# wanmeihuali/taichi_3d_gaussian_splatting

Hardware: NVIDIA B200
Metric: rendered Mpix/sec fwd+bwd @1080p, 1e6 Gaussians (higher is better)
Workload: dtype f32

## Files before the change

taichi_3d_gaussian_splatting_b200/csrc/api.cu:

```cuda
#include <cstdarg>
#include <cstdio>
#include <cstring>

#include "common.cuh"

namespace gsb {

static thread_local char g_error[512] = "";

void set_error(const char *fmt, ...) {
    va_list ap;
    va_start(ap, fmt);
    vsnprintf(g_error, sizeof(g_error), fmt, ap);
    va_end(ap);
}

static inline int64_t align_up(int64_t v, int64_t a) { return (v + a - 1) / a * a; }

static int bit_width(uint64_t v) {
    int b = 0;
    while (v) {
        ++b;
        v >>= 1;
    }
// ... 73 lines not shown
                      int32_t H, int32_t W, float far_plane, float depth_scale, uint32_t flags,
                      Workspace *ws) {
    int rc = compute_layout(N, n_obj, key_capacity, H, W, far_plane, depth_scale, flags, &ws->layout);
    if (rc != GSB_OK) return rc;
    const GsbWorkspaceLayout &L = ws->layout;
    if (!base || bytes < L.total_bytes) {
        set_error("workspace too small: have %lld bytes, need %lld", (long long)bytes, (long long)L.total_bytes);
        return GSB_EWORKSPACE;
    }
    if (reinterpret_cast<uintptr_t>(base) % 256 != 0) {
        set_error("workspace must be 256-byte aligned");
        return GSB_EINVAL;
    }
    char *b = static_cast<char *>(base);
    ws->counters = reinterpret_cast<long long *>(b + L.counters);
    ws->tickets = reinterpret_cast<unsigned int *>(b + L.tickets);
    ws->scan_state = reinterpret_cast<unsigned long long *>(b + L.scan_state);
    ws->sort_hist = reinterpret_cast<unsigned int *>(b + L.sort_hist);
    ws->sort_state = reinterpret_cast<unsigned int *>(b + L.sort_state);
    ws->tile_start = reinterpret_cast<int *>(b + L.tile_start);
    ws->tile_end = reinterpret_cast<int *>(b + L.tile_end);
    ws->poses = reinterpret_cast<PoseBlock *>(b + L.poses);
    ws->point_id = reinterpret_cast<int *>(b + L.point_id);
    ws->point_offset = reinterpret_cast<int *>(b + L.point_offset);
    ws->num_tiles = reinterpret_cast<int *>(b + L.num_tiles);
    ws->records = reinterpret_cast<float4 *>(b + L.records);
    ws->point_in_camera = reinterpret_cast<float *>(b + L.point_in_camera);
    ws->keys_a = b + L.keys_a;
    ws->keys_b = b + L.keys_b;
    ws->vals_a = reinterpret_cast<int *>(b + L.vals_a);
    ws->vals_b = reinterpret_cast<int *>(b + L.vals_b);
    ws->keys_c = b + L.keys_c;
    ws->vals_c = reinterpret_cast<int *>(b + L.vals_c);
    return GSB_OK;
}

static int check_forward_args(const GsbForwardArgs *a) {
    if (!a) {
        set_error("forward: args is null");
        return GSB_EINVAL;
    }
    if (a->num_points > 0 && (!a->pointcloud || !a->pointcloud_features || !a->point_invalid_mask ||
                              !a->point_object_id)) {
        set_error("forward: null scene pointer");
        return GSB_EINVAL;
    }
    if (a->num_points > 0 && (a->num_objects <= 0 || !a->q_pointcloud_camera || !a->t_pointcloud_camera)) {
        set_error("forward: need at least one object pose");
        return GSB_EINVAL;
    }
    if (!a->camera_intrinsics || !a->rasterized_image) {
        set_error("forward: null camera_intrinsics / rasterized_image");
        return GSB_EINVAL;
    }
    if (!a->rgb_only && (!a->rasterized_depth || !a->pixel_accumulated_alpha ||
                         !a->pixel_offset_of_last_effective_point || !a->pixel_valid_point_count)) {
        set_error("forward: aux outputs are required unless rgb_only");
        return GSB_EINVAL;
    }
    if (a->near_plane < 0.0f) {
        set_error("forward: near_plane must be >= 0 (depth keys are unsigned)");
        return GSB_EUNSUPPORTED;
    }
    if (reinterpret_cast<uintptr_t>(a->pointcloud_features) % 16 != 0) {
        set_error("forward: pointcloud_features must be 16-byte aligned");
        return GSB_EINVAL;
// ... 435 lines not shown
```

taichi_3d_gaussian_splatting_b200/csrc/blend_bwd.cu:

```cuda
#include "blend_bwd.cuh"

namespace gsb {

__device__ __forceinline__ void warp_transpose_reduce11(float (&v)[11], int lane) {
    {
        const bool hi = lane & 16;
#pragma unroll
        for (int i = 0; i < 5; ++i) {
            const float send = hi ? v[i] : v[i + 6];
            const float keep = hi ? v[i + 6] : v[i];
            v[i] = keep + __shfl_xor_sync(0xffffffffu, send, 16);
        }
        v[5] += __shfl_xor_sync(0xffffffffu, v[5], 16);
    }
    {
        const bool hi = lane & 8;
#pragma unroll
        for (int i = 0; i < 3; ++i) {
            const float send = hi ? v[i] : v[i + 3];
            const float keep = hi ? v[i + 3] : v[i];
            v[i] = keep + __shfl_xor_sync(0xffffffffu, send, 8);
        }
    }
    {
// ... 185 lines not shown
            }
        }
    }
    if (STATS) {
        p.mag_image[2 * pix] = mag0;
        p.mag_image[2 * pix + 1] = mag1;
    }
}

#ifndef GSB_HOST_EMU
static BlendBwdParams make_blend_bwd_params(const GsbBackwardArgs &a, const Workspace &ws);

int launch_blend_backward_work(const GsbBackwardArgs &a, const Workspace &ws, unsigned long long *counters_dev,
                               cudaStream_t stream) {
    BlendBwdParams p = make_blend_bwd_params(a, ws);
    p.work_counters = counters_dev;
    const int tiles = p.tiles_x * (a.camera_height / GSB_TILE_HEIGHT);
    if (tiles <= 0) return GSB_OK;
    return launch_blend_backward_count(p, tiles, stream);
}

static BlendBwdParams make_blend_bwd_params(const GsbBackwardArgs &a, const Workspace &ws) {
    BlendBwdParams p;
    p.H = a.camera_height;
    p.W = a.camera_width;
    p.tiles_x = a.camera_width / GSB_TILE_WIDTH;
    p.tile_start = ws.tile_start;
    p.tile_end = ws.tile_end;
    p.sorted_vals = ws.vals_b;
    p.records = ws.records;
    p.grad_image = a.grad_rasterized_image;
    p.acc_alpha = a.pixel_accumulated_alpha;
    p.last_effective = a.pixel_offset_of_last_effective_point;
    p.accum = a.accum;
    p.mag_image = a.magnitude_grad_viewspace_on_image;
    p.work_counters = nullptr;
    return p;
}

int launch_blend_backward(const GsbBackwardArgs &a, const Workspace &ws, cudaStream_t stream) {
    BlendBwdParams p;
    p.H = a.camera_height;
    p.W = a.camera_width;
    p.tiles_x = a.camera_width / GSB_TILE_WIDTH;
    p.tile_start = ws.tile_start;
    p.tile_end = ws.tile_end;
    p.sorted_vals = ws.vals_b;
    p.records = ws.records;
    p.grad_image = a.grad_rasterized_image;
    p.acc_alpha = a.pixel_accumulated_alpha;
    p.last_effective = a.pixel_offset_of_last_effective_point;
    p.accum = a.accum;
    p.mag_image = a.magnitude_grad_viewspace_on_image;
    p.work_counters = nullptr;
    const int tiles = p.tiles_x * (a.camera_height / GSB_TILE_HEIGHT);
    if (tiles <= 0) return GSB_OK;
    if (a.flags & GSB_FLAG_BACKWARD_TRANSPOSED)
        return launch_blend_backward_transposed(p, tiles, (a.flags & GSB_FLAG_EXACT_EXP) != 0,
                                                (a.flags & GSB_FLAG_NO_HOOK_STATS) == 0, stream);
    const bool exact = (a.flags & GSB_FLAG_EXACT_EXP) != 0;
    if (a.flags & GSB_FLAG_NO_HOOK_STATS) {
        if (exact) blend_backward_kernel<true, false><<<tiles, GSB_TILE_PIXELS, 0, stream>>>(p);
        else blend_backward_kernel<false, false><<<tiles, GSB_TILE_PIXELS, 0, stream>>>(p);
    } else if (exact) {
        blend_backward_kernel<true><<<tiles, GSB_TILE_PIXELS, 0, stream>>>(p);
    } else {
        blend_backward_kernel<false><<<tiles, GSB_TILE_PIXELS, 0, stream>>>(p);
    }
    GSB_CUDA_CHECK(cudaGetLastError());
    return GSB_OK;
}
#endif

__device__ __forceinline__ void sh_basis(float dx, float dy, float dz, float (&sh)[16]) {
    const float dinv = 1.0f / sqrtf(dx * dx + dy * dy + dz * dz);
    dx *= dinv; dy *= dinv; dz *= dinv;
    sh[0] = 0.28209479177387814f;
    sh[1] = -0.48860251190291987f * dy;
    sh[2] = 0.48860251190291987f * dz;
    sh[3] = -0.48860251190291987f * dx;
    sh[4] = 1.0925484305920792f * dx * dy;
    sh[5] = -1.0925484305920792f * dy * dz;
    sh[6] = 0.94617469575755997f * dz * dz - 0.31539156525251999f;
    sh[7] = -1.0925484305920792f * dx * dz;
// ... 368 lines not shown
```

taichi_3d_gaussian_splatting_b200/csrc/blend_bwd.cuh:

```cuda
#pragma once
#include "common.cuh"

namespace gsb {

struct BlendBwdParams {
    int H, W, tiles_x;
    const int *tile_start;
    const int *tile_end;
    const int *sorted_vals;
    const float4 *records;
    const float *grad_image;
    const float *acc_alpha;
    const int *last_effective;
    float *accum;
    float *mag_image;
    unsigned long long *work_counters;
};

#ifdef GSB_HOST_EMU
__device__ __forceinline__ float ex2_approx_b(float x) { return exp2f(x); }
__device__ __forceinline__ float rcp_approx(float x) { return 1.0f / x; }
__device__ __forceinline__ float sqrt_approx(float x) { return sqrtf(x); }
#else
__device__ __forceinline__ float ex2_approx_b(float x) {
    float y;
    asm("ex2.approx.ftz.f32 %0, %1;" : "=f"(y) : "f"(x));
    return y;
}
__device__ __forceinline__ float rcp_approx(float x) {
    float y;
    asm("rcp.approx.ftz.f32 %0, %1;" : "=f"(y) : "f"(x));
    return y;
}
__device__ __forceinline__ float sqrt_approx(float x) {
    float y;
    asm("sqrt.approx.ftz.f32 %0, %1;" : "=f"(y) : "f"(x));
    return y;
}
#endif

int launch_blend_backward_transposed(const BlendBwdParams &p, int tiles, bool exact_exp, bool stats,
                                     cudaStream_t stream);
int launch_blend_backward_count(const BlendBwdParams &p, int tiles, cudaStream_t stream);

}
```

taichi_3d_gaussian_splatting_b200/csrc/blend_bwd_transposed.cu:

```cuda
#include "blend_bwd.cuh"

namespace gsb {

constexpr int TB_CHUNK = 16;
constexpr int TB_ROW = TB_CHUNK + 1;
constexpr int TB_TR_ROW = 13;

struct TbShared {
    float4 rec[2 * 3 * GSB_TILE_PIXELS];
    float4 g[8][32];
    float xg[8][32 * TB_ROW];
    float xa[8][32 * TB_ROW];
    int off[2][GSB_TILE_PIXELS];
    float4 chunk[8][3][TB_CHUNK];
    int chunk_off[8][TB_CHUNK];
    unsigned int bits[2][8][8];
    unsigned char list[8][GSB_TILE_PIXELS];
    int max_last;
};
static_assert(32 * TB_ROW >= TB_CHUNK * TB_TR_ROW, "finished rows must fit into the exchange buffer");

#ifdef GSB_HOST_EMU
static inline unsigned char *tb_dynamic_smem() { return simt_emu::dynamic_smem(); }
#else
extern __shared__ __align__(16) unsigned char gsb_tb_dynamic_smem[];
__device__ __forceinline__ unsigned char *tb_dynamic_smem() { return gsb_tb_dynamic_smem; }
#endif

#ifndef GSB_TB_P1_UNROLL
#define GSB_TB_P1_UNROLL 4
#endif
constexpr int TB_P1_UNROLL = GSB_TB_P1_UNROLL;
#ifndef GSB_TB_MIN_BLOCKS
#define GSB_TB_MIN_BLOCKS 3
#endif
__device__ __forceinline__ float keep_if_contributing(float P, int idx, int last) {
#ifdef GSB_HOST_EMU
    return ((idx < last) && (P >= 1.0f / 255.0f)) ? P : 0.0f;
#else
    float r;
    asm("{\n"
        ".reg .pred p, q;\n"
        "setp.lt.s32 q, %2, %3;\n"
        "setp.ge.and.f32 p, %1, 0f3B808081, q;\n"
        "selp.f32 %0, %1, 0f00000000, p;\n"
        "}\n"
        : "=f"(r)
        : "f"(P), "r"(idx), "r"(last));
    return r;
#endif
}

template <bool EXACT_EXP, bool STATS, bool COUNT = false>
__global__ void __launch_bounds__(GSB_TILE_PIXELS, GSB_TB_MIN_BLOCKS)
blend_backward_transposed_kernel(const BlendBwdParams p) {
    TbShared &S = *reinterpret_cast<TbShared *>(tb_dynamic_smem());
    constexpr int NV = STATS ? 11 : 9;

    const int tile = blockIdx.x;
    const int tu = tile % p.tiles_x, tv = tile / p.tiles_x;
    const int tid = threadIdx.x, lane = tid & 31, warp = tid >> 5;
    const int pu = tu * GSB_TILE_WIDTH + (warp & 1) * 8 + (lane & 7);
    const int pv = tv * GSB_TILE_HEIGHT + (warp >> 1) * 4 + (lane >> 3);
    const float px = (float)pu + 0.5f, py = (float)pv + 0.5f;
    const float tile_x0 = (float)(tu * GSB_TILE_WIDTH), tile_y0 = (float)(tv * GSB_TILE_HEIGHT);
    const size_t pix = (size_t)pv * p.W + pu;
    const int start = p.tile_start[tile];

    const int last = p.last_effective[pix];
    float T = 1.0f - p.acc_alpha[pix];
    float w0 = 0.0f, w1 = 0.0f, w2 = 0.0f;
    const float g0 = p.grad_image[3 * pix], g1 = p.grad_image[3 * pix + 1], g2 = p.grad_image[3 * pix + 2];
    float mag0 = 0.0f, mag1 = 0.0f;
    unsigned int n_visits = 0, n_pairs = 0;
    S.g[warp][lane] = make_float4(g0, g1, g2, 0.0f);

    const int ci = lane & (TB_CHUNK - 1), half = lane >> 4;
    const float pxb = tile_x0 + (float)((warp & 1) * 8) + 0.5f;
    const float pyb = tile_y0 + (float)((warp >> 1) * 4 + 2 * half) + 0.5f;
    float *const xg = S.xg[warp], *const xa = S.xa[warp];
    const int fl_row = lane >= GSB_ACCUM_FLOATS ? 1 : 0;
    const int fl_word = lane - GSB_ACCUM_FLOATS * fl_row;
    const bool fl_ok = lane < 2 * GSB_ACCUM_FLOATS && fl_word < NV;
    const int *const fl_off = S.chunk_off[warp] + fl_row;
    const float *const fl_val = xg + fl_row * TB_TR_ROW + (fl_ok ? fl_word : 0);
    unsigned char *const list = S.list[warp];

    int warp_last = last;
#pragma unroll
    for (int d = 16; d > 0; d >>= 1) warp_last = max(warp_last, __shfl_xor_sync(0xffffffffu, warp_last, d));
    if (tid == 0) S.max_last = start;
    __syncthreads();
    if (lane == 0) atomicMax(&S.max_last, warp_last);
    __syncthreads();
    const int end = min(p.tile_end[tile], S.max_last);

    float4 *const ck0 = S.chunk[warp][0], *const ck1 = S.chunk[warp][1], *const ck2 = S.chunk[warp][2];
    int *const ck_off = S.chunk_off[warp];
    int have = 0;

    int buf = 0;
    for (int block_end = end;; block_end -= GSB_TILE_PIXELS, buf ^= 1) {
        const bool real = block_end > start;
        int count = 0;
        float4 *const s_r0 = S.rec + buf * 3 * GSB_TILE_PIXELS;
        float4 *const s_r1 = s_r0 + GSB_TILE_PIXELS, *const s_r2 = s_r0 + 2 * GSB_TILE_PIXELS;
        if (real) {
            const int block_start = max(block_end - GSB_TILE_PIXELS, start);
            {
                const int idx = block_end - 1 - tid;
                unsigned int mask = 0;
                if (idx >= block_start) {
                    const int o = __ldg(&p.sorted_vals[idx]);
                    const float4 *rec = p.records + 3 * (size_t)o;
                    const float4 r0 = __ldg(rec), r1 = __ldg(rec + 1);
                    if (EXACT_EXP) {
                        s_r0[tid] = r0;
                        s_r1[tid] = r1;
                    } else {
                        float4 f0, f1;
                        fast_planes(r0, r1, f0, f1);
                        s_r0[tid] = f0;
                        s_r1[tid] = f1;
                    }
                    s_r2[tid] = __ldg(rec + 2);
                    S.off[buf][tid] = o;
                    mask = splat_patch_mask(r0.x, r0.y, r0.z, r0.w, r1.x, r1.y * r1.z, tile_x0, tile_y0);
                }
#pragma unroll
                for (int w = 0; w < 8; ++w) {
                    const unsigned int bits = __ballot_sync(0xffffffffu, (mask >> w) & 1u);
                    if (lane == 0) S.bits[buf][w][warp] = bits;
                }
            }
            __syncthreads();
            if (tid == 0) GSB_EMU_COUNT(EC_BATCHES, 1);
            if (block_start < warp_last) {
                const int skip = block_end - warp_last;
#pragma unroll
                for (int k = 0; k < 8; ++k) {
                    unsigned int bits = S.bits[buf][warp][k];
                    const int lo = skip - 32 * k;
                    if (lo >= 32) bits = 0u;
                    else if (lo > 0) bits &= ~((1u << lo) - 1u);
                    if ((bits >> lane) & 1u)
                        list[count + __popc(bits & ((1u << lane) - 1u))] = (unsigned char)(k * 32 + lane);
                    count += __popc(bits);
                }
                __syncwarp();
            }
        }

        int pos = 0;
#pragma unroll 1
        do {
            if (pos < count) {
                const int take = min(TB_CHUNK - have, count - pos);
                if (lane < take) {
                    const int j = list[pos + lane], slot = have + lane;
                    ck0[slot] = s_r0[j];
                    ck1[slot] = s_r1[j];
                    float4 r2 = s_r2[j];
                    r2.w = __int_as_float(block_end - 1 - j);
                    ck2[slot] = r2;
                    ck_off[slot] = S.off[buf][j];
                }
                have += take;
                pos += take;
                __syncwarp();
            }
            if (have == TB_CHUNK || (!real && have > 0)) {
                const int n = have;
                have = 0;
                if (COUNT) n_visits += (lane == 0) ? (unsigned int)n : 0u;
                if (lane == 0) {
                    GSB_EMU_COUNT(EC_TB_SPLATS, n);
                    GSB_EMU_COUNT(EC_TB_CHUNKS, 1);
                }
#pragma unroll TB_P1_UNROLL
                for (int i = 0; i < n; ++i) {
                    const float4 r0 = ck0[i];
                    const float4 r1 = ck1[i];
                    const float4 r2 = ck2[i];
                    const int idx = __float_as_int(r2.w);
                    const float d0 = px - r0.x, d1 = py - r0.y;
                    float G, aT;
                    if (EXACT_EXP) {
                        const float q0 = r0.z * d0 + r0.w * d1;
                        const float q1 = r0.w * d0 + r1.x * d1;
                        const float gp = expf(-0.5f * (d0 * q0 + d1 * q1)) * r1.y;
                        const float prod_alpha = gp * r1.z;
                        const bool contributes = (idx < last) && (prod_alpha >= 1.0f / 255.0f);
                        const float alpha = fminf(prod_alpha, 0.99f);
                        const float inv = 1.0f / (1.0f - alpha);
                        const float Tn = T * inv;
                        aT = contributes ? alpha * Tn : 0.0f;
                        const float a_grad = contributes ? (r2.x * Tn - w0 * inv) * g0 + (r2.y * Tn - w1 * inv) * g1 +
                                                               (r2.z * Tn - w2 * inv) * g2
                                                         : 0.0f;
                        T = contributes ? Tn : T;
                        w0 = fmaf(r2.x, aT, w0);
                        w1 = fmaf(r2.y, aT, w1);
                        w2 = fmaf(r2.z, aT, w2);
                        G = a_grad * r1.z * gp;
                        if (STATS) {
                            mag0 += fabsf(G * q0);
                            mag1 += fabsf(G * q1);
                        }
                    } else {
                        float P = fast_alpha(d0, d1, r0.z, r0.w, r1.x, r1.y);
                        P = keep_if_contributing(P, idx, last);
                        const float alpha = fminf(P, 0.99f);
                        const float inv = rcp_approx(1.0f - alpha);
                        T *= inv;
                        aT = alpha * T;
                        const float cg = fmaf(r2.z, g2, fmaf(r2.y, g1, r2.x * g0));
                        const float a_grad = fmaf(cg, T, -(w0 * inv));
                        w0 = fmaf(cg, aT, w0);
                        G = a_grad * P;
                        if (STATS) {
                            const float q0 = (-2.0f / GSB_L2E) * fmaf(r0.z, d0, 0.5f * r0.w * d1);
                            const float q1 = (-2.0f / GSB_L2E) * fmaf(0.5f * r0.w, d0, r1.x * d1);
                            mag0 += fabsf(G * q0);
                            mag1 += fabsf(G * q1);
                        }
                    }
                    if (COUNT) n_pairs += aT > 0.0f ? 1u : 0u;
                    xg[lane * TB_ROW + i] = G;
                    xa[lane * TB_ROW + i] = aT;
                }
                __syncwarp();

                const bool active = ci < n;
                float4 s0 = ck0[active ? ci : 0];
                float4 s1 = ck1[active ? ci : 0];
                if (!EXACT_EXP) {
                    s0.z *= -2.0f / GSB_L2E;
                    s0.w *= -1.0f / GSB_L2E;
                    s1.x *= -2.0f / GSB_L2E;
                }
                const float dx0 = pxb - s0.x;
                float acc[11];
#pragma unroll
                for (int k = 0; k < 11; ++k) acc[k] = 0.0f;
                unsigned int nz = 0u;
#pragma unroll
                for (int row = 0; row < 2; ++row) {
                    const float d1 = (pyb + (float)row) - s0.y;
                    float q0 = s0.z * dx0 + s0.w * d1;
                    float q1 = s0.w * dx0 + s1.x * d1;
#pragma unroll
                    for (int k = 0; k < 8; ++k) {
                        const int pp = 8 * row + k + 16 * half;
                        const float G = xg[pp * TB_ROW + ci], aT = xa[pp * TB_ROW + ci];
                        const float4 gp = S.g[warp][pp];
                        const float vs0 = G * q0, vs1 = G * q1;
                        acc[0] += vs0;
                        acc[1] += vs1;
                        acc[2] = fmaf(vs0, q0, acc[2]);
                        acc[3] = fmaf(vs0, q1, acc[3]);
                        acc[4] = fmaf(vs1, q1, acc[4]);
                        acc[5] = fmaf(aT, gp.x, acc[5]);
                        acc[6] = fmaf(aT, gp.y, acc[6]);
                        acc[7] = fmaf(aT, gp.z, acc[7]);
                        acc[8] += G;
                        if (STATS) {
                            const float m2 = vs0 * vs0 + vs1 * vs1;
                            acc[9] += EXACT_EXP ? sqrtf(m2) : sqrt_approx(m2);
                            acc[10] += aT > 0.0f ? 1.0f : 0.0f;
                        }
                        nz |= __float_as_uint(aT);
                        q0 += s0.z;
                        q1 += s0.w;
                    }
                }
#pragma unroll
                for (int k = 0; k < NV; ++k) acc[k] += __shfl_xor_sync(0xffffffffu, acc[k], 16);
                nz |= __shfl_xor_sync(0xffffffffu, nz, 16);
                acc[8] *= EXACT_EXP ? (1.0f - s1.z) : s1.z;
                __syncwarp();
                if (lane < TB_CHUNK) {
                    if (!(active && nz != 0u)) ck_off[ci] = -1;
                    else GSB_EMU_COUNT(EC_TB_ROWS, 1);
#pragma unroll
                    for (int k = 0; k < NV; ++k) xg[ci * TB_TR_ROW + k] = acc[k];
                }
                __syncwarp();
#pragma unroll
                for (int step = 0; step < TB_CHUNK / 2; ++step) {
                    const int o = fl_off[2 * step];
                    const float v = fl_val[2 * step * TB_TR_ROW];
                    if (fl_ok && o >= 0) atomicAdd(p.accum + (size_t)o * GSB_ACCUM_FLOATS + fl_word, v);
                }
                __syncwarp();
            }
        } while (pos < count);
        if (!real) break;
    }
    if (STATS) {
        p.mag_image[2 * pix] = mag0;
        p.mag_image[2 * pix + 1] = mag1;
    }
    if (COUNT) {
#pragma unroll
        for (int d = 16; d > 0; d >>= 1) {
            n_visits += __shfl_xor_sync(0xffffffffu, n_visits, d);
            n_pairs += __shfl_xor_sync(0xffffffffu, n_pairs, d);
        }
        if (lane == 0) {
            atomicAdd(p.work_counters, (unsigned long long)n_visits);
            atomicAdd(p.work_counters + 1, (unsigned long long)n_pairs);
        }
    }
}

#ifndef GSB_HOST_EMU
template <bool EXACT_EXP, bool STATS>
static int launch_tb(const BlendBwdParams &p, int tiles, cudaStream_t stream) {
    static bool configured = false;
    if (!configured) {
        GSB_CUDA_CHECK(cudaFuncSetAttribute(blend_backward_transposed_kernel<EXACT_EXP, STATS>,
                                            cudaFuncAttributeMaxDynamicSharedMemorySize, (int)sizeof(TbShared)));
        configured = true;
    }
    blend_backward_transposed_kernel<EXACT_EXP, STATS><<<tiles, GSB_TILE_PIXELS, sizeof(TbShared), stream>>>(p);
    GSB_CUDA_CHECK(cudaGetLastError());
    return GSB_OK;
}

int launch_blend_backward_transposed(const BlendBwdParams &p, int tiles, bool exact_exp, bool stats,
// ... 16 lines not shown
```

taichi_3d_gaussian_splatting_b200/csrc/blend_fwd.cu:

```cuda
#include "common.cuh"

namespace gsb {

struct BlendFwdParams {
    int H, W, tiles_x;
    const int *tile_start;
    const int *tile_end;
    const int *sorted_vals;
    const float4 *records;
    float *image;
    float *depth;
    float *acc_alpha;
    int *last_effective;
    int *valid_count;
    unsigned long long *work_counters;
};

__device__ __forceinline__ float ex2_approx(float x) { return ex2_mufu(x); }

__device__ __forceinline__ void count_if_blended(float wgt, int idx, int &cnt, int &last) {
#ifdef GSB_HOST_EMU
    if (wgt > 0.0f) {
        cnt += 1;
        last = idx;
    }
#else
    asm("{\n"
        ".reg .pred p;\n"
        "setp.gt.f32 p, %2, 0f00000000;\n"
        "@p add.s32 %0, %0, 1;\n"
        "@p mov.b32 %1, %3;\n"
        "}\n"
        : "+r"(cnt), "+r"(last)
        : "f"(wgt), "r"(idx));
#endif
}

#ifndef GSB_FWD_MIN_BLOCKS
#define GSB_FWD_MIN_BLOCKS 4
#endif
#ifndef GSB_FWD_UNROLL
#define GSB_FWD_UNROLL 8
#endif
constexpr int FW_UNROLL = GSB_FWD_UNROLL;
constexpr int FW_CHUNK = 32;

template <bool RGB_ONLY, bool EXACT_EXP, bool COUNT = false>
__global__ void __launch_bounds__(GSB_TILE_PIXELS, GSB_FWD_MIN_BLOCKS)
blend_forward_kernel(const BlendFwdParams p) {
    __shared__ float4 s_rec[2 * 3 * GSB_TILE_PIXELS];
    __shared__ unsigned int s_bits[2][8][8];
// ... 8 lines not shown
    const float px = (float)pu + 0.5f, py = (float)pv + 0.5f;
    const float tile_x0 = (float)(tu * GSB_TILE_WIDTH), tile_y0 = (float)(tv * GSB_TILE_HEIGHT);
    const int start = p.tile_start[tile], end = p.tile_end[tile];

    float T = 1.0f, Tlive = 1.0f, C0 = 0.0f, C1 = 0.0f, C2 = 0.0f, D = 0.0f, Wt = 0.0f;
    int last = start, cnt = 0;
    unsigned int n_visits = 0, n_pairs = 0;
    unsigned int n_p84 = 0, n_p88 = 0, n_p164 = 0, n_p44 = 0;
    float4 *const ck0 = s_chunk[warp][0], *const ck1 = s_chunk[warp][1], *const ck2 = s_chunk[warp][2];
    unsigned char *const list = s_list[warp];
    const unsigned int lt_mask = (1u << lane) - 1u;

    int buf = 0;
    for (int base = start; base < end; base += GSB_TILE_PIXELS, buf ^= 1) {
        float4 *const s_r0 = s_rec + buf * 3 * GSB_TILE_PIXELS;
        float4 *const s_r1 = s_r0 + GSB_TILE_PIXELS, *const s_r2 = s_r0 + 2 * GSB_TILE_PIXELS;
        const int idx = base + tid;
        unsigned int mask = 0;
        if (idx < end) {
            const int o = __ldg(&p.sorted_vals[idx]);
            const float4 *rec = p.records + 3 * (size_t)o;
            const float4 r0 = __ldg(rec), r1 = __ldg(rec + 1);
            if (EXACT_EXP) {
                s_r0[tid] = r0;
                s_r1[tid] = r1;
            } else {
                float4 f0, f1;
                fast_planes(r0, r1, f0, f1);
                s_r0[tid] = f0;
                s_r1[tid] = f1;
            }
            s_r2[tid] = __ldg(rec + 2);
            mask = splat_patch_mask(r0.x, r0.y, r0.z, r0.w, r1.x, r1.y * r1.z, tile_x0, tile_y0);
            if (COUNT) {
                n_p84 += __popc(mask);
                n_p88 += __popc((mask | (mask >> 2)) & 0x33u);
                n_p164 += __popc((mask | (mask >> 1)) & 0x55u);
                const SplatReach rr = make_splat_reach(r0.z, r0.w, r1.x, r1.y * r1.z);
                if (rr.mode == 2) n_p44 += 16;
                else if (rr.mode == 1)
                    for (int q = 0; q < 16; ++q) {
                        const float X0 = tile_x0 + 4.0f * (q & 3) + 0.5f - r0.x, Y0 = tile_y0 + 4.0f * (q >> 2) + 0.5f - r0.y;
                        n_p44 += rect_reachable(rr, X0, X0 + 3.0f, Y0, Y0 + 3.0f) ? 1 : 0;
                    }
            }
        }
#pragma unroll
        for (int w = 0; w < 8; ++w) {
            const unsigned int bits = __ballot_sync(0xffffffffu, (mask >> w) & 1u);
            if (lane == 0) s_bits[buf][w][warp] = bits;
        }
        if (__syncthreads_and(!(T > 0.0f))) break;
        if (__all_sync(0xffffffffu, !(T > 0.0f))) continue;
        int count = 0;
#pragma unroll
        for (int k = 0; k < 8; ++k) {
            const unsigned int bits = s_bits[buf][warp][k];
            if ((bits >> lane) & 1u) list[count + __popc(bits & lt_mask)] = (unsigned char)(k * 32 + lane);
            count += __popc(bits);
        }
        __syncwarp();
#pragma unroll 1
        for (int pos = 0; pos < count; pos += FW_CHUNK) {
            const int n = min(FW_CHUNK, count - pos);
            if (lane < n) {
                const int j = list[pos + lane];
// ... 76 lines not shown
            n_visits += __shfl_xor_sync(0xffffffffu, n_visits, d);
            n_pairs += __shfl_xor_sync(0xffffffffu, n_pairs, d);
            n_p84 += __shfl_xor_sync(0xffffffffu, n_p84, d);
            n_p88 += __shfl_xor_sync(0xffffffffu, n_p88, d);
            n_p164 += __shfl_xor_sync(0xffffffffu, n_p164, d);
            n_p44 += __shfl_xor_sync(0xffffffffu, n_p44, d);
        }
        if (lane == 0) {
            atomicAdd(p.work_counters, (unsigned long long)n_visits);
            atomicAdd(p.work_counters + 1, (unsigned long long)n_pairs);
            atomicAdd(p.work_counters + 2, (unsigned long long)n_p84);
            atomicAdd(p.work_counters + 3, (unsigned long long)n_p88);
            atomicAdd(p.work_counters + 4, (unsigned long long)n_p164);
            atomicAdd(p.work_counters + 5, (unsigned long long)n_p44);
        }
    }
}

#ifndef GSB_HOST_EMU
int launch_blend_forward(const GsbForwardArgs &a, const Workspace &ws, cudaStream_t stream) {
    BlendFwdParams p;
    p.H = a.camera_height;
    p.W = a.camera_width;
    p.tiles_x = a.camera_width / GSB_TILE_WIDTH;
    p.tile_start = ws.tile_start;
    p.tile_end = ws.tile_end;
    p.sorted_vals = ws.vals_b;
    p.records = ws.records;
    p.image = a.rasterized_image;
    p.depth = a.rasterized_depth;
    p.acc_alpha = a.pixel_accumulated_alpha;
    p.last_effective = a.pixel_offset_of_last_effective_point;
    p.valid_count = a.pixel_valid_point_count;
    p.work_counters = nullptr;
    const int tiles = p.tiles_x * (a.camera_height / GSB_TILE_HEIGHT);
    if (tiles <= 0) return GSB_OK;
    const bool exact = (a.flags & GSB_FLAG_EXACT_EXP) != 0;
    if (a.rgb_only) {
        if (exact) blend_forward_kernel<true, true><<<tiles, GSB_TILE_PIXELS, 0, stream>>>(p);
        else blend_forward_kernel<true, false><<<tiles, GSB_TILE_PIXELS, 0, stream>>>(p);
    } else {
        if (exact) blend_forward_kernel<false, true><<<tiles, GSB_TILE_PIXELS, 0, stream>>>(p);
        else blend_forward_kernel<false, false><<<tiles, GSB_TILE_PIXELS, 0, stream>>>(p);
    }
    GSB_CUDA_CHECK(cudaGetLastError());
    return GSB_OK;
}

int launch_blend_forward_count(const GsbForwardArgs &a, const Workspace &ws, unsigned long long *counters_dev,
                               cudaStream_t stream) {
    BlendFwdParams p;
    p.H = a.camera_height;
    p.W = a.camera_width;
    p.tiles_x = a.camera_width / GSB_TILE_WIDTH;
    p.tile_start = ws.tile_start;
    p.tile_end = ws.tile_end;
    p.sorted_vals = ws.vals_b;
    p.records = ws.records;
    p.image = a.rasterized_image;
    p.depth = a.rasterized_depth;
    p.acc_alpha = a.pixel_accumulated_alpha;
    p.last_effective = a.pixel_offset_of_last_effective_point;
    p.valid_count = a.pixel_valid_point_count;
    p.work_counters = counters_dev;
    const int tiles = p.tiles_x * (a.camera_height / GSB_TILE_HEIGHT);
    if (tiles <= 0) return GSB_OK;
    blend_forward_kernel<false, false, true><<<tiles, GSB_TILE_PIXELS, 0, stream>>>(p);
    GSB_CUDA_CHECK(cudaGetLastError());
    return GSB_OK;
}
#endif

}
```

taichi_3d_gaussian_splatting_b200/csrc/common.cuh:

```cuda
#pragma once
#include <cuda_runtime.h>
#include <stdint.h>

#include "../../include/gsb200.h"

#define GSB_TILE_PIXELS (GSB_TILE_WIDTH * GSB_TILE_HEIGHT)

namespace gsb {

void set_error(const char *fmt, ...);
#define GSB_CUDA_CHECK(expr)                                                                   \
    do {                                                                                       \
        cudaError_t _e = (expr);                                                               \
        if (_e != cudaSuccess) {                                                               \
            gsb::set_error("%s failed: %s (%s:%d)", #expr, cudaGetErrorString(_e), __FILE__,   \
                           __LINE__);                                                          \
            return GSB_ECUDA;                                                                  \
        }                                                                                      \
    } while (0)

enum Counter { CNT_M = 0, CNT_K = 1, CNT_OVERFLOW = 2, CNT_MAX_DEPTH_KEY = 4 };
enum Ticket { TICKET_SCAN = 0, TICKET_SORT0 = 1  };

struct PoseBlock {
    float T[12];
    float centre[3];
    float pad[5];
};
static_assert(sizeof(PoseBlock) == 80, "PoseBlock layout");

struct Workspace {
    long long *counters;
    unsigned int *tickets;
    unsigned long long *scan_state;
    unsigned int *sort_hist;
    unsigned int *sort_state;
    int *tile_start;
    int *tile_end;
    PoseBlock *poses;
    int *point_id;
    int *point_offset;
    int *num_tiles;
    float4 *records;
    float *point_in_camera;
    void *keys_a, *keys_b, *keys_c;
    int *vals_a, *vals_b, *vals_c;
    GsbWorkspaceLayout layout;
};

int resolve_workspace(void *base, int64_t bytes, int64_t N, int32_t n_obj, int64_t key_capacity,
                      int32_t H, int32_t W, float far_plane, float depth_scale, uint32_t flags,
                      Workspace *ws);

int launch_preprocess(const GsbForwardArgs &a, const Workspace &ws, cudaStream_t stream);
int launch_sort(const Workspace &ws, int64_t key_capacity, cudaStream_t stream);
int launch_tile_ranges(const Workspace &ws, int64_t key_capacity, int num_tiles, cudaStream_t stream);
int launch_tile_ranges_raw(const long long *keys_i64, int64_t n, int *tile_start, int *tile_end,
                           int num_tiles, cudaStream_t stream);
int launch_blend_forward(const GsbForwardArgs &a, const Workspace &ws, cudaStream_t stream);
int launch_blend_backward(const GsbBackwardArgs &a, const Workspace &ws, cudaStream_t stream);
int launch_backward_points(const GsbBackwardArgs &a, const Workspace &ws, cudaStream_t stream,
                           const long long *skip_flag = nullptr);
int launch_adam_step(float *param, const float *grad, float *exp_avg, float *exp_avg_sq, long long n, double lr, double beta1,
                     double beta2, double eps, int step, const long long *skip_flag, cudaStream_t stream);
int launch_expand_view_gradients(const GsbExpandArgs &a, cudaStream_t stream);
int launch_blend_forward_count(const GsbForwardArgs &a, const Workspace &ws, unsigned long long *counters_dev,
                               cudaStream_t stream);
int launch_blend_backward_work(const GsbBackwardArgs &a, const Workspace &ws, unsigned long long *counters_dev,
                               cudaStream_t stream);

int sort_radix_bits(int bits);
int sort_pairs_device(const void *keys_in, const int *vals_in, void *keys_out, int *vals_out,
                      const long long *n_dev, int64_t n_capacity, int key_bytes, int depth_bits, int end_bit,
                      const int *max_depth_key , unsigned int *hist ,
                      unsigned int *state , unsigned int *tickets , void *tmp_keys,
                      int *tmp_vals, cudaStream_t stream);

#ifndef GSB_SORT_ITEMS
#define GSB_SORT_ITEMS 12
// ... 91 lines not shown
    return m;
}
#endif

#if defined(__CUDACC__) || defined(GSB_HOST_EMU)
constexpr float GSB_L2E = 1.4426950408889634f;
#ifdef GSB_HOST_EMU
__device__ __forceinline__ float ex2_mufu(float x) { return exp2f(x); }
#else
__device__ __forceinline__ float ex2_mufu(float x) {
    float y;
    asm("ex2.approx.ftz.f32 %0, %1;" : "=f"(y) : "f"(x));
    return y;
}
#endif
__device__ __forceinline__ float fast_alpha(float dx, float dy, float A, float B, float C, float ro) {
    return ex2_mufu(fmaf(dx, fmaf(A, dx, B * dy), (C * dy) * dy)) * ro;
}
__device__ __forceinline__ void fast_planes(const float4 r0, const float4 r1, float4 &s0, float4 &s1) {
    s0 = make_float4(r0.x, r0.y, (-0.5f * GSB_L2E) * r0.z, -GSB_L2E * r0.w);
    s1 = make_float4((-0.5f * GSB_L2E) * r1.x, r1.y * r1.z, 1.0f - r1.z, r1.w);
}
#endif

#if defined(__CUDACC__) || defined(GSB_HOST_EMU)
#ifdef GSB_HOST_EMU
__device__ __forceinline__ void mbar_init(unsigned long long *bar, unsigned int) { *bar = 0; }
__device__ __forceinline__ void mbar_arrive_expect_tx(unsigned long long *, unsigned int) {}
__device__ __forceinline__ void bulk_copy_g2s(void *dst_smem, const void *src_gmem, unsigned int bytes,
                                              unsigned long long *) {
    memcpy(dst_smem, src_gmem, bytes);
}
__device__ __forceinline__ void mbar_wait(unsigned long long *, unsigned int) { simt_emu::warp_exchange(0u); }
#else
__device__ __forceinline__ unsigned int smem_addr(const void *p) {
    return (unsigned int)__cvta_generic_to_shared(p);
}
__device__ __forceinline__ void mbar_init(unsigned long long *bar, unsigned int count) {
    asm volatile("mbarrier.init.shared::cta.b64 [%0], %1;" ::"r"(smem_addr(bar)), "r"(count));
    asm volatile("fence.mbarrier_init.release.cluster;" ::: "memory");
}
__device__ __forceinline__ void mbar_arrive_expect_tx(unsigned long long *bar, unsigned int bytes) {
    asm volatile("mbarrier.arrive.expect_tx.shared::cta.b64 _, [%0], %1;" ::"r"(smem_addr(bar)),
                 "r"(bytes)
                 : "memory");
}
__device__ __forceinline__ void bulk_copy_g2s(void *dst_smem, const void *src_gmem, unsigned int bytes,
                                              unsigned long long *bar) {
    asm volatile(
        "cp.async.bulk.shared::cluster.global.mbarrier::complete_tx::bytes [%0], [%1], %2, [%3];" ::"r"(
            smem_addr(dst_smem)),
        "l"(src_gmem), "r"(bytes), "r"(smem_addr(bar))
        : "memory");
}
__device__ __forceinline__ void mbar_wait(unsigned long long *bar, unsigned int parity) {
    asm volatile(
        "{\n"
        ".reg .pred p;\n"
        "WAIT_LOOP:\n"
        "mbarrier.try_wait.parity.shared::cta.b64 p, [%0], %1;\n"
        "@p bra WAIT_DONE;\n"
        "bra WAIT_LOOP;\n"
        "WAIT_DONE:\n"
        "}\n" ::"r"(smem_addr(bar)),
        "r"(parity)
        : "memory");
}
#endif

#endif

#ifdef GSB_HOST_EMU
#define GSB_EMU_COUNT(slot, n) (simt_emu::counters()[slot] += (long long)(n))
#else
#define GSB_EMU_COUNT(slot, n) ((void)0)
#endif
enum EmuCounter {
    EC_BF_VISITS = 0,
    EC_BF_VISITS_ANY = 1,
    EC_BF_PAIRS = 2,
    EC_TB_SPLATS = 3,
    EC_TB_CHUNKS = 4,
    EC_TB_ROWS = 5,
    EC_BATCHES = 6,
    EC_FW_VISITS = 7,
    EC_FW_PAIRS = 8,
};

static inline int num_sms() {
    static int n = 0;
    if (n == 0) {
        int dev = 0;
        cudaGetDevice(&dev);
        cudaDeviceGetAttribute(&n, cudaDevAttrMultiProcessorCount, dev);
        if (n <= 0) n = 148;
    }
    return n;
}

}
```

Before: 1416.

## Reuse forward patch masks in transposed backward with per-warp cp.async double buffering

The forward blend kernel now writes each sorted splat's 8-bit patch mask into the workspace, reusing the keys_c region. The transposed backward kernel reads these masks instead of recomputing them. Each warp builds its own chunk list directly from global memory with a ballot scan, and chunk records are prefetched into double-buffered shared memory with cp.async, so the block-wide staging, __syncthreads and max_last reduction go away. Smaller shared memory allows raising min blocks per SM to 4 for the fast-exp path, at the cost of more register pressure, per-warp redundant scanning, and reliance on keys_c being free between forward and backward.

```diff
diff --git a/taichi_3d_gaussian_splatting_b200/csrc/api.cu b/taichi_3d_gaussian_splatting_b200/csrc/api.cu
--- a/taichi_3d_gaussian_splatting_b200/csrc/api.cu
+++ b/taichi_3d_gaussian_splatting_b200/csrc/api.cu
@@ -129,6 +129,7 @@
     ws->vals_b = reinterpret_cast<int *>(b + L.vals_b);
     ws->keys_c = b + L.keys_c;
     ws->vals_c = reinterpret_cast<int *>(b + L.vals_c);
+    ws->patch_masks = reinterpret_cast<unsigned char *>(b + L.keys_c);
     return GSB_OK;
 }
 
diff --git a/taichi_3d_gaussian_splatting_b200/csrc/blend_bwd.cu b/taichi_3d_gaussian_splatting_b200/csrc/blend_bwd.cu
--- a/taichi_3d_gaussian_splatting_b200/csrc/blend_bwd.cu
+++ b/taichi_3d_gaussian_splatting_b200/csrc/blend_bwd.cu
@@ -241,6 +241,7 @@
     p.grad_image = a.grad_rasterized_image;
     p.acc_alpha = a.pixel_accumulated_alpha;
     p.last_effective = a.pixel_offset_of_last_effective_point;
+    p.patch_masks = ws.patch_masks;
     p.accum = a.accum;
     p.mag_image = a.magnitude_grad_viewspace_on_image;
     p.work_counters = nullptr;
@@ -259,6 +260,7 @@
     p.grad_image = a.grad_rasterized_image;
     p.acc_alpha = a.pixel_accumulated_alpha;
     p.last_effective = a.pixel_offset_of_last_effective_point;
+    p.patch_masks = ws.patch_masks;
     p.accum = a.accum;
     p.mag_image = a.magnitude_grad_viewspace_on_image;
     p.work_counters = nullptr;
diff --git a/taichi_3d_gaussian_splatting_b200/csrc/blend_bwd.cuh b/taichi_3d_gaussian_splatting_b200/csrc/blend_bwd.cuh
--- a/taichi_3d_gaussian_splatting_b200/csrc/blend_bwd.cuh
+++ b/taichi_3d_gaussian_splatting_b200/csrc/blend_bwd.cuh
@@ -12,6 +12,7 @@
     const float *grad_image;
     const float *acc_alpha;
     const int *last_effective;
+    const unsigned char *patch_masks = nullptr;
     float *accum;
     float *mag_image;
     unsigned long long *work_counters;
diff --git a/taichi_3d_gaussian_splatting_b200/csrc/blend_bwd_transposed.cu b/taichi_3d_gaussian_splatting_b200/csrc/blend_bwd_transposed.cu
--- a/taichi_3d_gaussian_splatting_b200/csrc/blend_bwd_transposed.cu
+++ b/taichi_3d_gaussian_splatting_b200/csrc/blend_bwd_transposed.cu
@@ -7,16 +7,12 @@
 constexpr int TB_TR_ROW = 13;
 
 struct TbShared {
-    float4 rec[2 * 3 * GSB_TILE_PIXELS];
     float4 g[8][32];
     float xg[8][32 * TB_ROW];
     float xa[8][32 * TB_ROW];
-    int off[2][GSB_TILE_PIXELS];
-    float4 chunk[8][3][TB_CHUNK];
-    int chunk_off[8][TB_CHUNK];
-    unsigned int bits[2][8][8];
-    unsigned char list[8][GSB_TILE_PIXELS];
-    int max_last;
+    float4 chunk[8][2][3][TB_CHUNK];
+    int chunk_off[8][2][TB_CHUNK];
+    int chunk_idx[8][2][TB_CHUNK];
 };
 static_assert(32 * TB_ROW >= TB_CHUNK * TB_TR_ROW, "finished rows must fit into the exchange buffer");
 
@@ -32,8 +28,9 @@
 #endif
 constexpr int TB_P1_UNROLL = GSB_TB_P1_UNROLL;
 #ifndef GSB_TB_MIN_BLOCKS
-#define GSB_TB_MIN_BLOCKS 3
-#endif
+#define GSB_TB_MIN_BLOCKS 4
+#endif
+constexpr int tb_min_blocks(bool exact_exp) { return exact_exp && GSB_TB_MIN_BLOCKS > 3 ? 3 : GSB_TB_MIN_BLOCKS; }
 __device__ __forceinline__ float keep_if_contributing(float P, int idx, int last) {
 #ifdef GSB_HOST_EMU
     return ((idx < last) && (P >= 1.0f / 255.0f)) ? P : 0.0f;
@@ -51,8 +48,20 @@
 #endif
 }
 
+#ifdef GSB_HOST_EMU
+inline unsigned int load_patch_mask(const BlendBwdParams &p, int i, float tile_x0, float tile_y0) {
+    if (p.patch_masks) return p.patch_masks[i];
+    const float4 *r = p.records + 3 * (size_t)p.sorted_vals[i];
+    return splat_patch_mask(r[0].x, r[0].y, r[0].z, r[0].w, r[1].x, r[1].y * r[1].z, tile_x0, tile_y0);
+}
+#else
+__device__ __forceinline__ unsigned int load_patch_mask(const BlendBwdParams &p, int i, float, float) {
+    return __ldg(p.patch_masks + i);
+}
+#endif
+
 template <bool EXACT_EXP, bool STATS, bool COUNT = false>
-__global__ void __launch_bounds__(GSB_TILE_PIXELS, GSB_TB_MIN_BLOCKS)
+__global__ void __launch_bounds__(GSB_TILE_PIXELS, tb_min_blocks(EXACT_EXP))
 blend_backward_transposed_kernel(const BlendBwdParams p) {
     TbShared &S = *reinterpret_cast<TbShared *>(tb_dynamic_smem());
     constexpr int NV = STATS ? 11 : 9;
@@ -82,220 +91,205 @@
     const int fl_row = lane >= GSB_ACCUM_FLOATS ? 1 : 0;
     const int fl_word = lane - GSB_ACCUM_FLOATS * fl_row;
     const bool fl_ok = lane < 2 * GSB_ACCUM_FLOATS && fl_word < NV;
-    const int *const fl_off = S.chunk_off[warp] + fl_row;
     const float *const fl_val = xg + fl_row * TB_TR_ROW + (fl_ok ? fl_word : 0);
-    unsigned char *const list = S.list[warp];
-
     int warp_last = last;
 #pragma unroll
     for (int d = 16; d > 0; d >>= 1) warp_last = max(warp_last, __shfl_xor_sync(0xffffffffu, warp_last, d));
-    if (tid == 0) S.max_last = start;
-    __syncthreads();
-    if (lane == 0) atomicMax(&S.max_last, warp_last);
-    __syncthreads();
-    const int end = min(p.tile_end[tile], S.max_last);
-
-    float4 *const ck0 = S.chunk[warp][0], *const ck1 = S.chunk[warp][1], *const ck2 = S.chunk[warp][2];
-    int *const ck_off = S.chunk_off[warp];
-    int have = 0;
+
+    const unsigned int bit = 1u << warp;
+    const unsigned int lt_mask = (1u << lane) - 1u;
+    int top = warp_last + 32;
+    unsigned int sel = 0u;
+    int val = 0;
+    unsigned int next_mask = 0u;
+    int next_val = 0;
+    {
+        const int i = warp_last - 1 - lane;
+        if (i >= start) {
+            next_mask = load_patch_mask(p, i, tile_x0, tile_y0);
+            next_val = __ldg(p.sorted_vals + i);
+        }
+    }
+    auto fill = [&](int b) -> int {
+        float4 *const c0 = S.chunk[warp][b][0], *const c1 = S.chunk[warp][b][1], *const c2 = S.chunk[warp][b][2];
+        int have = 0;
+        while (have < TB_CHUNK) {
+            if (sel == 0u) {
+                top -= 32;
+                if (top <= start) break;
+                if (lane == 0) GSB_EMU_COUNT(EC_TB_WINDOWS, 1);
+                const int i = top - 1 - lane;
+                sel = __ballot_sync(0xffffffffu, i >= start && (next_mask & bit) != 0u);
+                val = next_val;
+                next_mask = 0u;
+                if (i - 32 >= start) {
+                    next_mask = load_patch_mask(p, i - 32, tile_x0, tile_y0);
+                    next_val = __ldg(p.sorted_vals + i - 32);
+                }
+                continue;
+            }
+            const int take = min(__popc(sel), TB_CHUNK - have);
+            const int rank = __popc(sel & lt_mask);
+            const bool mine = (sel >> lane) & 1u;
+            if (mine && rank < take) {
+                const int slot = have + rank;
+                const float4 *rec = p.records + 3 * (size_t)val;
+                cp_async16(c0 + slot, rec);
+                cp_async16(c1 + slot, rec + 1);
+                cp_async16(c2 + slot, rec + 2);
+                S.chunk_off[warp][b][slot] = val;
+                S.chunk_idx[warp][b][slot] = top - 1 - lane;
+            }
+            sel = take == TB_CHUNK - have ? __ballot_sync(0xffffffffu, mine && rank >= take) : 0u;
+            have += take;
+        }
+        cp_async_commit();
+        return have;
+    };
 
     int buf = 0;
-    for (int block_end = end;; block_end -= GSB_TILE_PIXELS, buf ^= 1) {
-        const bool real = block_end > start;
-        int count = 0;
-        float4 *const s_r0 = S.rec + buf * 3 * GSB_TILE_PIXELS;
-        float4 *const s_r1 = s_r0 + GSB_TILE_PIXELS, *const s_r2 = s_r0 + 2 * GSB_TILE_PIXELS;
-        if (real) {
-            const int block_start = max(block_end - GSB_TILE_PIXELS, start);
-            {
-                const int idx = block_end - 1 - tid;
-                unsigned int mask = 0;
-                if (idx >= block_start) {
-                    const int o = __ldg(&p.sorted_vals[idx]);
-                    const float4 *rec = p.records + 3 * (size_t)o;
-                    const float4 r0 = __ldg(rec), r1 = __ldg(rec + 1);
-                    if (EXACT_EXP) {
-                        s_r0[tid] = r0;
-                        s_r1[tid] = r1;
-                    } else {
-                        float4 f0, f1;
-                        fast_planes(r0, r1, f0, f1);
-                        s_r0[tid] = f0;
-                        s_r1[tid] = f1;
-                    }
-                    s_r2[tid] = __ldg(rec + 2);
-                    S.off[buf][tid] = o;
-                    mask = splat_patch_mask(r0.x, r0.y, r0.z, r0.w, r1.x, r1.y * r1.z, tile_x0, tile_y0);
+    int n = fill(0);
+#pragma unroll 1
+    while (n > 0) {
+        const int n_next = fill(buf ^ 1);
+        cp_async_wait<1>();
+        __syncwarp();
+        float4 *const ck0 = S.chunk[warp][buf][0], *const ck1 = S.chunk[warp][buf][1], *const ck2 = S.chunk[warp][buf][2];
+        int *const ck_off = S.chunk_off[warp][buf];
+        const int *const fl_off = ck_off + fl_row;
+        if (lane < n) {
+            if (!EXACT_EXP) {
+                float4 f0, f1;
+                fast_planes(ck0[lane], ck1[lane], f0, f1);
+                ck0[lane] = f0;
+                ck1[lane] = f1;
+            }
+            ck2[lane].w = __int_as_float(S.chunk_idx[warp][buf][lane]);
+        }
+        __syncwarp();
+        if (COUNT) n_visits += (lane == 0) ? (unsigned int)n : 0u;
+        if (lane == 0) {
+            GSB_EMU_COUNT(EC_TB_SPLATS, n);
+            GSB_EMU_COUNT(EC_TB_CHUNKS, 1);
+        }
+#pragma unroll TB_P1_UNROLL
+        for (int i = 0; i < n; ++i) {
+            const float4 r0 = ck0[i];
+            const float4 r1 = ck1[i];
+            const float4 r2 = ck2[i];
+            const int idx = __float_as_int(r2.w);
+            const float d0 = px - r0.x, d1 = py - r0.y;
+            float G, aT;
+            if (EXACT_EXP) {
+                const float q0 = r0.z * d0 + r0.w * d1;
+                const float q1 = r0.w * d0 + r1.x * d1;
+                const float gp = expf(-0.5f * (d0 * q0 + d1 * q1)) * r1.y;
+                const float prod_alpha = gp * r1.z;
+                const bool contributes = (idx < last) && (prod_alpha >= 1.0f / 255.0f);
+                const float alpha = fminf(prod_alpha, 0.99f);
+                const float inv = 1.0f / (1.0f - alpha);
+                const float Tn = T * inv;
+                aT = contributes ? alpha * Tn : 0.0f;
+                const float a_grad = contributes ? (r2.x * Tn - w0 * inv) * g0 + (r2.y * Tn - w1 * inv) * g1 +
+                                                       (r2.z * Tn - w2 * inv) * g2
+                                                 : 0.0f;
+                T = contributes ? Tn : T;
+                w0 = fmaf(r2.x, aT, w0);
+                w1 = fmaf(r2.y, aT, w1);
+                w2 = fmaf(r2.z, aT, w2);
+                G = a_grad * r1.z * gp;
+                if (STATS) {
+                    mag0 += fabsf(G * q0);
+                    mag1 += fabsf(G * q1);
                 }
-#pragma unroll
-                for (int w = 0; w < 8; ++w) {
-                    const unsigned int bits = __ballot_sync(0xffffffffu, (mask >> w) & 1u);
-                    if (lane == 0) S.bits[buf][w][warp] = bits;
+            } else {
+                float P = fast_alpha(d0, d1, r0.z, r0.w, r1.x, r1.y);
+                P = keep_if_contributing(P, idx, last);
+                const float alpha = fminf(P, 0.99f);
+                const float inv = rcp_approx(1.0f - alpha);
+                T *= inv;
+                aT = alpha * T;
+                const float cg = fmaf(r2.z, g2, fmaf(r2.y, g1, r2.x * g0));
+                const float a_grad = fmaf(cg, T, -(w0 * inv));
+                w0 = fmaf(cg, aT, w0);
+                G = a_grad * P;
+                if (STATS) {
+                    const float q0 = (-2.0f / GSB_L2E) * fmaf(r0.z, d0, 0.5f * r0.w * d1);
+                    const float q1 = (-2.0f / GSB_L2E) * fmaf(0.5f * r0.w, d0, r1.x * d1);
+                    mag0 += fabsf(G * q0);
+                    mag1 += fabsf(G * q1);
                 }
             }
-            __syncthreads();
-            if (tid == 0) GSB_EMU_COUNT(EC_BATCHES, 1);
-            if (block_start < warp_last) {
-                const int skip = block_end - warp_last;
-#pragma unroll
-                for (int k = 0; k < 8; ++k) {
-                    unsigned int bits = S.bits[buf][warp][k];
-                    const int lo = skip - 32 * k;
-                    if (lo >= 32) bits = 0u;
-                    else if (lo > 0) bits &= ~((1u << lo) - 1u);
-                    if ((bits >> lane) & 1u)
-                        list[count + __popc(bits & ((1u << lane) - 1u))] = (unsigned char)(k * 32 + lane);
-                    count += __popc(bits);
+            if (COUNT) n_pairs += aT > 0.0f ? 1u : 0u;
+            xg[lane * TB_ROW + i] = G;
+            xa[lane * TB_ROW + i] = aT;
+        }
+        __syncwarp();
+
+        const bool active = ci < n;
+        float4 s0 = ck0[active ? ci : 0];
+        float4 s1 = ck1[active ? ci : 0];
+        if (!EXACT_EXP) {
+            s0.z *= -2.0f / GSB_L2E;
+            s0.w *= -1.0f / GSB_L2E;
+            s1.x *= -2.0f / GSB_L2E;
+        }
+        const float dx0 = pxb - s0.x;
+        float acc[11];
+#pragma unroll
+        for (int k = 0; k < 11; ++k) acc[k] = 0.0f;
+        unsigned int nz = 0u;
+#pragma unroll
+        for (int row = 0; row < 2; ++row) {
+            const float d1 = (pyb + (float)row) - s0.y;
+            float q0 = s0.z * dx0 + s0.w * d1;
+            float q1 = s0.w * dx0 + s1.x * d1;
+#pragma unroll
+            for (int k = 0; k < 8; ++k) {
+                const int pp = 8 * row + k + 16 * half;
+                const float G = xg[pp * TB_ROW + ci], aT = xa[pp * TB_ROW + ci];
+                const float4 gp = S.g[warp][pp];
+                const float vs0 = G * q0, vs1 = G * q1;
+                acc[0] += vs0;
+                acc[1] += vs1;
+                acc[2] = fmaf(vs0, q0, acc[2]);
+                acc[3] = fmaf(vs0, q1, acc[3]);
+                acc[4] = fmaf(vs1, q1, acc[4]);
+                acc[5] = fmaf(aT, gp.x, acc[5]);
+                acc[6] = fmaf(aT, gp.y, acc[6]);
+                acc[7] = fmaf(aT, gp.z, acc[7]);
+                acc[8] += G;
+                if (STATS) {
+                    const float m2 = vs0 * vs0 + vs1 * vs1;
+                    acc[9] += EXACT_EXP ? sqrtf(m2) : sqrt_approx(m2);
+                    acc[10] += aT > 0.0f ? 1.0f : 0.0f;
                 }
-                __syncwarp();
-            }
-        }
-
-        int pos = 0;
-#pragma unroll 1
-        do {
-            if (pos < count) {
-                const int take = min(TB_CHUNK - have, count - pos);
-                if (lane < take) {
-                    const int j = list[pos + lane], slot = have + lane;
-                    ck0[slot] = s_r0[j];
-                    ck1[slot] = s_r1[j];
-                    float4 r2 = s_r2[j];
-                    r2.w = __int_as_float(block_end - 1 - j);
-                    ck2[slot] = r2;
-                    ck_off[slot] = S.off[buf][j];
-                }
-                have += take;
-                pos += take;
-                __syncwarp();
-            }
-            if (have == TB_CHUNK || (!real && have > 0)) {
-                const int n = have;
-                have = 0;
-                if (COUNT) n_visits += (lane == 0) ? (unsigned int)n : 0u;
-                if (lane == 0) {
-                    GSB_EMU_COUNT(EC_TB_SPLATS, n);
-                    GSB_EMU_COUNT(EC_TB_CHUNKS, 1);
-                }
-#pragma unroll TB_P1_UNROLL
-                for (int i = 0; i < n; ++i) {
-                    const float4 r0 = ck0[i];
-                    const float4 r1 = ck1[i];
-                    const float4 r2 = ck2[i];
-                    const int idx = __float_as_int(r2.w);
-                    const float d0 = px - r0.x, d1 = py - r0.y;
-                    float G, aT;
-                    if (EXACT_EXP) {
-                        const float q0 = r0.z * d0 + r0.w * d1;
-                        const float q1 = r0.w * d0 + r1.x * d1;
-                        const float gp = expf(-0.5f * (d0 * q0 + d1 * q1)) * r1.y;
-                        const float prod_alpha = gp * r1.z;
-                        const bool contributes = (idx < last) && (prod_alpha >= 1.0f / 255.0f);
-                        const float alpha = fminf(prod_alpha, 0.99f);
-                        const float inv = 1.0f / (1.0f - alpha);
-                        const float Tn = T * inv;
-                        aT = contributes ? alpha * Tn : 0.0f;
-                        const float a_grad = contributes ? (r2.x * Tn - w0 * inv) * g0 + (r2.y * Tn - w1 * inv) * g1 +
-                                                               (r2.z * Tn - w2 * inv) * g2
-                                                         : 0.0f;
-                        T = contributes ? Tn : T;
-                        w0 = fmaf(r2.x, aT, w0);
-                        w1 = fmaf(r2.y, aT, w1);
-                        w2 = fmaf(r2.z, aT, w2);
-                        G = a_grad * r1.z * gp;
-                        if (STATS) {
-                            mag0 += fabsf(G * q0);
-                            mag1 += fabsf(G * q1);
-                        }
-                    } else {
-                        float P = fast_alpha(d0, d1, r0.z, r0.w, r1.x, r1.y);
-                        P = keep_if_contributing(P, idx, last);
-                        const float alpha = fminf(P, 0.99f);
-                        const float inv = rcp_approx(1.0f - alpha);
-                        T *= inv;
-                        aT = alpha * T;
-                        const float cg = fmaf(r2.z, g2, fmaf(r2.y, g1, r2.x * g0));
-                        const float a_grad = fmaf(cg, T, -(w0 * inv));
-                        w0 = fmaf(cg, aT, w0);
-                        G = a_grad * P;
-                        if (STATS) {
-                            const float q0 = (-2.0f / GSB_L2E) * fmaf(r0.z, d0, 0.5f * r0.w * d1);
-                            const float q1 = (-2.0f / GSB_L2E) * fmaf(0.5f * r0.w, d0, r1.x * d1);
-                            mag0 += fabsf(G * q0);
-                            mag1 += fabsf(G * q1);
-                        }
-                    }
-                    if (COUNT) n_pairs += aT > 0.0f ? 1u : 0u;
-                    xg[lane * TB_ROW + i] = G;
-                    xa[lane * TB_ROW + i] = aT;
-                }
-                __syncwarp();
-
-                const bool active = ci < n;
-                float4 s0 = ck0[active ? ci : 0];
-                float4 s1 = ck1[active ? ci : 0];
-                if (!EXACT_EXP) {
-                    s0.z *= -2.0f / GSB_L2E;
-                    s0.w *= -1.0f / GSB_L2E;
-                    s1.x *= -2.0f / GSB_L2E;
-                }
-                const float dx0 = pxb - s0.x;
-                float acc[11];
-#pragma unroll
-                for (int k = 0; k < 11; ++k) acc[k] = 0.0f;
-                unsigned int nz = 0u;
-#pragma unroll
-                for (int row = 0; row < 2; ++row) {
-                    const float d1 = (pyb + (float)row) - s0.y;
-                    float q0 = s0.z * dx0 + s0.w * d1;
-                    float q1 = s0.w * dx0 + s1.x * d1;
-#pragma unroll
-                    for (int k = 0; k < 8; ++k) {
-                        const int pp = 8 * row + k + 16 * half;
-                        const float G = xg[pp * TB_ROW + ci], aT = xa[pp * TB_ROW + ci];
-                        const float4 gp = S.g[warp][pp];
-                        const float vs0 = G * q0, vs1 = G * q1;
-                        acc[0] += vs0;
-                        acc[1] += vs1;
-                        acc[2] = fmaf(vs0, q0, acc[2]);
-                        acc[3] = fmaf(vs0, q1, acc[3]);
-                        acc[4] = fmaf(vs1, q1, acc[4]);
-                        acc[5] = fmaf(aT, gp.x, acc[5]);
-                        acc[6] = fmaf(aT, gp.y, acc[6]);
-                        acc[7] = fmaf(aT, gp.z, acc[7]);
-                        acc[8] += G;
-                        if (STATS) {
-                            const float m2 = vs0 * vs0 + vs1 * vs1;
-                            acc[9] += EXACT_EXP ? sqrtf(m2) : sqrt_approx(m2);
-                            acc[10] += aT > 0.0f ? 1.0f : 0.0f;
-                        }
-                        nz |= __float_as_uint(aT);
-                        q0 += s0.z;
-                        q1 += s0.w;
-                    }
-                }
-#pragma unroll
-                for (int k = 0; k < NV; ++k) acc[k] += __shfl_xor_sync(0xffffffffu, acc[k], 16);
-                nz |= __shfl_xor_sync(0xffffffffu, nz, 16);
-                acc[8] *= EXACT_EXP ? (1.0f - s1.z) : s1.z;
-                __syncwarp();
-                if (lane < TB_CHUNK) {
-                    if (!(active && nz != 0u)) ck_off[ci] = -1;
-                    else GSB_EMU_COUNT(EC_TB_ROWS, 1);
-#pragma unroll
-                    for (int k = 0; k < NV; ++k) xg[ci * TB_TR_ROW + k] = acc[k];
-                }
-                __syncwarp();
-#pragma unroll
-                for (int step = 0; step < TB_CHUNK / 2; ++step) {
-                    const int o = fl_off[2 * step];
-                    const float v = fl_val[2 * step * TB_TR_ROW];
-                    if (fl_ok && o >= 0) atomicAdd(p.accum + (size_t)o * GSB_ACCUM_FLOATS + fl_word, v);
-                }
-                __syncwarp();
-            }
-        } while (pos < count);
-        if (!real) break;
+                nz |= __float_as_uint(aT);
+                q0 += s0.z;
+                q1 += s0.w;
+            }
+        }
+#pragma unroll
+        for (int k = 0; k < NV; ++k) acc[k] += __shfl_xor_sync(0xffffffffu, acc[k], 16);
+        nz |= __shfl_xor_sync(0xffffffffu, nz, 16);
+        acc[8] *= EXACT_EXP ? (1.0f - s1.z) : s1.z;
+        __syncwarp();
+        if (lane < TB_CHUNK) {
+            if (!(active && nz != 0u)) ck_off[ci] = -1;
+            else GSB_EMU_COUNT(EC_TB_ROWS, 1);
+#pragma unroll
+            for (int k = 0; k < NV; ++k) xg[ci * TB_TR_ROW + k] = acc[k];
+        }
+        __syncwarp();
+#pragma unroll
+        for (int step = 0; step < TB_CHUNK / 2; ++step) {
+            const int o = fl_off[2 * step];
+            const float v = fl_val[2 * step * TB_TR_ROW];
+            if (fl_ok && o >= 0) atomicAdd(p.accum + (size_t)o * GSB_ACCUM_FLOATS + fl_word, v);
+        }
+        __syncwarp();
+        buf ^= 1;
+        n = n_next;
     }
     if (STATS) {
         p.mag_image[2 * pix] = mag0;
diff --git a/taichi_3d_gaussian_splatting_b200/csrc/blend_fwd.cu b/taichi_3d_gaussian_splatting_b200/csrc/blend_fwd.cu
--- a/taichi_3d_gaussian_splatting_b200/csrc/blend_fwd.cu
+++ b/taichi_3d_gaussian_splatting_b200/csrc/blend_fwd.cu
@@ -13,10 +13,21 @@
     float *acc_alpha;
     int *last_effective;
     int *valid_count;
+    unsigned char *patch_masks = nullptr;
     unsigned long long *work_counters;
 };
 
 __device__ __forceinline__ float ex2_approx(float x) { return ex2_mufu(x); }
+
+#ifdef GSB_HOST_EMU
+inline void store_patch_mask(unsigned char *masks, int idx, unsigned int mask) {
+    if (masks) masks[idx] = (unsigned char)mask;
+}
+#else
+__device__ __forceinline__ void store_patch_mask(unsigned char *masks, int idx, unsigned int mask) {
+    masks[idx] = (unsigned char)mask;
+}
+#endif
 
 __device__ __forceinline__ void count_if_blended(float wgt, int idx, int &cnt, int &last) {
 #ifdef GSB_HOST_EMU
@@ -91,6 +102,7 @@
             }
             s_r2[tid] = __ldg(rec + 2);
             mask = splat_patch_mask(r0.x, r0.y, r0.z, r0.w, r1.x, r1.y * r1.z, tile_x0, tile_y0);
+            if (!RGB_ONLY) store_patch_mask(p.patch_masks, idx, mask);
             if (COUNT) {
                 n_p84 += __popc(mask);
                 n_p88 += __popc((mask | (mask >> 2)) & 0x33u);
@@ -233,6 +245,7 @@
     p.acc_alpha = a.pixel_accumulated_alpha;
     p.last_effective = a.pixel_offset_of_last_effective_point;
     p.valid_count = a.pixel_valid_point_count;
+    p.patch_masks = ws.patch_masks;
     p.work_counters = nullptr;
     const int tiles = p.tiles_x * (a.camera_height / GSB_TILE_HEIGHT);
     if (tiles <= 0) return GSB_OK;
@@ -263,6 +276,7 @@
     p.acc_alpha = a.pixel_accumulated_alpha;
     p.last_effective = a.pixel_offset_of_last_effective_point;
     p.valid_count = a.pixel_valid_point_count;
+    p.patch_masks = ws.patch_masks;
     p.work_counters = counters_dev;
     const int tiles = p.tiles_x * (a.camera_height / GSB_TILE_HEIGHT);
     if (tiles <= 0) return GSB_OK;
diff --git a/taichi_3d_gaussian_splatting_b200/csrc/common.cuh b/taichi_3d_gaussian_splatting_b200/csrc/common.cuh
--- a/taichi_3d_gaussian_splatting_b200/csrc/common.cuh
+++ b/taichi_3d_gaussian_splatting_b200/csrc/common.cuh
@@ -45,6 +45,7 @@
     float *point_in_camera;
     void *keys_a, *keys_b, *keys_c;
     int *vals_a, *vals_b, *vals_c;
+    unsigned char *patch_masks;
     GsbWorkspaceLayout layout;
 };
 
@@ -202,6 +203,10 @@
     memcpy(dst_smem, src_gmem, bytes);
 }
 __device__ __forceinline__ void mbar_wait(unsigned long long *, unsigned int) { simt_emu::warp_exchange(0u); }
+__device__ __forceinline__ void cp_async16(void *dst_smem, const void *src_gmem) { memcpy(dst_smem, src_gmem, 16); }
+__device__ __forceinline__ void cp_async_commit() {}
+template <int N>
+__device__ __forceinline__ void cp_async_wait() { simt_emu::warp_exchange(0u); }
 #else
 __device__ __forceinline__ unsigned int smem_addr(const void *p) {
     return (unsigned int)__cvta_generic_to_shared(p);
@@ -236,6 +241,14 @@
         "r"(parity)
         : "memory");
 }
+__device__ __forceinline__ void cp_async16(void *dst_smem, const void *src_gmem) {
+    asm volatile("cp.async.ca.shared.global [%0], [%1], 16;" ::"r"(smem_addr(dst_smem)), "l"(src_gmem) : "memory");
+}
+__device__ __forceinline__ void cp_async_commit() { asm volatile("cp.async.commit_group;" ::: "memory"); }
+template <int N>
+__device__ __forceinline__ void cp_async_wait() {
+    asm volatile("cp.async.wait_group %0;" ::"n"(N) : "memory");
+}
 #endif
 
 #endif
@@ -252,7 +265,7 @@
     EC_TB_SPLATS = 3,
     EC_TB_CHUNKS = 4,
     EC_TB_ROWS = 5,
-    EC_BATCHES = 6,
+    EC_TB_WINDOWS = 6,
     EC_FW_VISITS = 7,
     EC_FW_PAIRS = 8,
 };
```

Result: faster. 1502, median of 6 (+6.1%).
